# abstract-liu/LORB_SLAM

Hardware: AMD Instinct MI355X
Metric: ORB matches/sec + local-BA iterations/sec (50 KF, 10k pts) at 1/2/4/8 MI355X (higher is better)
Workload: dtype f64+u8; 1 GPU; c4_local_mapping_step_chained; windows_per_gpu=1, kf=50, fixed_kf=5, points=10679, observations=75130, new_kf_keypoints=2000, match=2000x~10679 bf crossCheck, parallelism=independent windows x1

## Files before the change

### lorb_slam_amd/csrc/lorb_ba.hip

```cpp
#ifndef LORB_NO_CONTRACT
#pragma clang fp contract(fast)
#endif
#include "lorb_ba_math.h"
#include "lorb_internal.h"
#include "lorb_ba_dev.h"
#include "lorb_ba_plan.h"

#include <algorithm>
#include <cmath>
#include <type_traits>

namespace {

using namespace lorb::ba;
using lorb::residual;
using lorb::residual_jac;
using lorb::residual_jac_s;
using lorb::residual_s;

__device__ __forceinline__ void init_run(const BaDev& d, int W, int ctot, int n_pt, int nf, const LMOpt& o, const int i,
                                         const int stride) {
  if (i < W) {
    WinState s;
    s.radius = o.init_radius; s.decrease_factor = 2.0; s.cost = 0.0; s.x_norm = 0.0; s.gmax = 0.0;
// ... 1453 lines not shown
    const int n = std::max(std::max(std::max(P->W, P->Ctot), P->NF), std::min(3 * P->pt_launch, 256 * 1024));
    hipLaunchKernelGGL(k_ba_init, dim3(lorb::ceil_div(std::max(n, 1), 256)), dim3(256), 0, ctx->stream, P->dev, P->W,
                       P->Ctot, P->pt_launch, P->NF, o);
  }
  LORB_CHECK_LAUNCH(ctx);
  if (o.max_iter <= 0) return enqueue_linearize(P, o);
  for (int it = 0; it < o.max_iter; ++it) LORB_TRY(enqueue_iteration(P, o, it == 0, it + 1 == o.max_iter));
  return LORB_OK;
}

int plan_solve(lorb_ba_plan* P, const lorb_lm_options* opt) {
  lorb_ctx* ctx = P->ctx;
  LMOpt o = to_dev_opt(opt);
  P->fold = fold_of(P);
  const bool timing = ctx->ktime || no_graph() || (P->comm && !P->comm->rccl);
  if (timing) return enqueue_solve(P, o);
  const lorb_ba_plan::GraphKey key = graph_key(P);
  const bool same = key == P->gkey && same_opt(P->graph_opt, o);
  return P->cache.replay_or_capture(ctx, same, [&] { return enqueue_solve(P, o); },
                                    [&] { P->gkey = key; P->graph_opt = o; });
}

int plan_read(lorb_ba_plan* P, double* const* pose_out, double* const* point_out,
              lorb_ba_summary* sums) {
  lorb_ctx* ctx = P->ctx;
  std::vector<WinState> st(P->W);
  std::vector<std::vector<double>> hp(P->W);
  LORB_HIP(ctx, hipMemcpyAsync(st.data(), P->d_state, sizeof(WinState) * P->W, hipMemcpyDeviceToHost, ctx->stream));
  LORB_HIP(ctx, hipStreamSynchronize(ctx->stream));
  for (int w = 0; w < P->W; ++w) {
    const BaWin& bw = P->hwin[w];
    const int cur = st[w].cur;
// ... 10 lines not shown
      if (bw.n_obs_all == 0) { s.iterations = 0; s.termination = LORB_TERM_FUNCTION_TOL; }
      sums[w] = s;
    }
  }
  LORB_HIP(ctx, hipStreamSynchronize(ctx->stream));
  for (int w = 0; w < P->W; ++w) {
    if (hp[w].empty()) continue;
    const std::vector<int>& map = P->cam_map[w];
    for (int c = 0; c < P->hwin[w].n_poses; ++c)
      for (int q = 0; q < 6; ++q)
        pose_out[w][6 * (size_t)c + q] = hp[w][6 * (size_t)(map.empty() ? c : map[c]) + q];
  }
  return LORB_OK;
}

}

struct lorb_ba_group {
  lorb_ctx* ctx = nullptr;
  std::vector<lorb_ba_plan*> plans;
  GraphCache cache{"group graph"};
  LMOpt graph_opt{};
  std::vector<unsigned> gens;
  std::vector<lorb_ba_plan::GraphKey> keys;
  int n_fused = 0;
};

namespace {

bool group_fused(const lorb_ba_group* G) {
// ... 343 lines not shown
```

### lorb_slam_amd/csrc/lorb_ba_build.hip

```cpp
#ifndef LORB_NO_CONTRACT
#pragma clang fp contract(fast)
#endif
#include "lorb_ba_math.h"
#include "lorb_internal.h"
#include "lorb_ba_dev.h"
#include "lorb_ba_plan.h"

#include <algorithm>
#include <chrono>
#include <cmath>
#include <map>

struct lorb_ba_devbuild {
  int K_cap = 0, P_cap = 0, C = 0, F = 0, Wd = 0;
  int* key_out = nullptr; int* val_out = nullptr;
  int* scr = nullptr; size_t scr_bytes = 0;
  int* pt_cnt = nullptr;
  int* hdr = nullptr;
  int* cov = nullptr;
  int* cam_cnt = nullptr;
  unsigned long long* bits = nullptr;
  int* perm = nullptr;
  int pblk_cap = 0, part_cap = 0, gspan_cap = 0, sgrp_cap = 0;
  size_t gpart_cap = 0;
  int* pinned = nullptr; size_t pinned_n = 0;
  bool dirty = true;
  bool sorted_hint = false;
  std::vector<double> h_red;
  unsigned char* up_dev = nullptr; unsigned char* up_host = nullptr; int up_bp_cap = 0;
  const unsigned char* up_host_dev = nullptr;
  size_t off_live = 0, off_perm = 0, off_gcam = 0, off_bp = 0, up_bytes = 0;
  std::vector<char> last_adj;
  std::vector<int> h_copy;
  std::vector<int> last_map;
  hipEvent_t rb_ev = nullptr;
  bool rb_pending = false, rb_sorted = false, rb_fuse = false;
  ~lorb_ba_devbuild() {
    if (rb_ev) (void)hipEventDestroy(rb_ev);
    if (pinned) (void)hipHostFree(pinned);
    if (up_host) (void)hipHostFree(up_host);
  }
};

namespace {

using namespace lorb::ba;

void print_diagnostics(const lorb_ba_plan& p) {
  if (p.hp_n)
// ... 715 lines not shown
    const unsigned long long bal = __ballot(pr);
    const unsigned msk = half ? (unsigned)(bal >> 32) : (unsigned)bal;
    if (n > 0) {
      if (msk) {
        const int f = __builtin_ctz(msk);
        hi = lo + (int)(((long long)n * (f + 1)) / 33);
        if (f > 0) lo = lo + (int)(((long long)n * f) / 33) + 1;
      } else {
        lo = lo + (int)(((long long)n * 32) / 33) + 1;
      }
    }
  }
  s0 = __shfl(lo, 0, 64);
  s1 = __shfl(lo, 32, 64);
}
__global__ __launch_bounds__(256) void k_db_gather(lorb_ba_window_dev w, BaDev d, int K, const int* __restrict__ key,
                                                   const int* __restrict__ val, DbFused f, DbCams cams) {
  const int gt = blockIdx.x * 256 + threadIdx.x, gs = gridDim.x * 256;
  for (int i = gt; i < f.up_words; i += gs) f.up_dst[i] = f.up_src[i];
  const int* __restrict__ perm = cams.perm;
  const int* __restrict__ gcam = cams.gcam;
  {
    const int m = max(max(6 * f.C, 6 * f.F), 3 * f.P);
    for (int i = gt; i < m; i += gs) {
      if (i < 6 * f.C) {
        const int c = i / 6, q = i - 6 * c;
        d.x_init_pose[6 * perm[c] + q] = (double)w.d_pose_init[i];
        if (q == 0) const_cast<int*>(d.cam_active)[perm[c]] = gcam[c] > 0;
      }
      if (i < 6 * f.F) const_cast<double*>(d.fixed_pose)[i] = (double)w.d_fixed_pose[i];
      if (i < 3 * f.P) d.x_init_pt[i] = (double)w.d_point_init[i];
    }
  }
  for (int g = gt >> 6; g < f.G; g += gs >> 6) {
    int s0, s1;
    group_bounds(d.pt_obs_off, f.P, (long long)g * f.S, (long long)(g + 1) * f.S, threadIdx.x & 63, s0, s1);
    if ((threadIdx.x & 63) == 0) {
      PBlk b;
      b.win = 0; b.p0 = s0; b.cnt = s1 - s0; b.o0 = d.pt_obs_off[s0]; b.no = d.pt_obs_off[s1] - d.pt_obs_off[s0];
      const_cast<PBlk*>(d.pblk)[g] = b;
    }
  }
  for (int i = gt; i < f.nsg; i += gs) f.sgrp[i] = make_int4(0, i * f.sgf, min(f.sgf, f.G - i * f.sgf), 0);
// ... 101 lines not shown
  P->hwin.assign(1, BaWin{});
  P->pt_launch = b.P_cap;
  return LORB_OK;
}

int up_alloc(lorb_ba_plan* P, int bp_need) {
  lorb_ba_devbuild& b = *P->devb;
  if (b.up_dev && b.up_bp_cap >= bp_need) return LORB_OK;
  lorb_ctx* ctx = P->ctx;
  const int cap = std::max(bp_need + bp_need / 4, 16);
  auto al = [](size_t x) { return (x + 255) & ~(size_t)255; };
  const size_t C = (size_t)std::max(b.C, 1);
  b.off_live = al(sizeof(BaWin));
  b.off_perm = b.off_live + 256;
  b.off_gcam = b.off_perm + al(4 * C);
  b.off_bp = b.off_gcam + al(4 * C);
  b.up_bytes = b.off_bp + sizeof(BlockPair) * (size_t)cap;
  if (b.up_dev) {
    LORB_TRY(dfree(P, b.up_dev));
    (void)hipHostFree(b.up_host);
    b.up_host = nullptr;
  }
  LORB_TRY(dalloc(P, b.up_bytes, &b.up_dev));
  LORB_HIP(ctx, hipHostMalloc(reinterpret_cast<void**>(&b.up_host), b.up_bytes));
  LORB_HIP(ctx, hipHostGetDevicePointer((void**)&b.up_host_dev, b.up_host, 0));
  b.up_bp_cap = cap;
  BaDev& d = P->dev;
  d.win = reinterpret_cast<const BaWin*>(b.up_dev);
  d.live = reinterpret_cast<const int*>(b.up_dev + b.off_live);
  b.perm = reinterpret_cast<int*>(b.up_dev + b.off_perm);
  d.bp = reinterpret_cast<const BlockPair*>(b.up_dev + b.off_bp);
  P->grid_bp = cap;
// ... 140 lines not shown
                           shape_ok ? "another rank" : "this rank", w->n_poses, b.C, w->n_fixed, b.F);
  if (gerr & 64)
    return phase_rc != LORB_OK ? phase_rc
                               : lorb::set_error(ctx, LORB_E_DEVICE, "device plan build failed on another rank");
  if (gerr & 8) return lorb::set_error(ctx, LORB_E_INVALID, "live point / observation count outside [0, capacity] (%d / %d)",
                                       b.P_cap, b.K_cap);
  if (gerr & 1) return lorb::set_error(ctx, LORB_E_INVALID, "observation with a point index outside [0, n_points)");
  if (gerr & 2) return lorb::set_error(ctx, LORB_E_INVALID, "observation with a frame index >= n_poses");
  if (gerr & 4) return lorb::set_error(ctx, LORB_E_INVALID, "a point observed twice by one camera");
  if ((gerr & 16) || Pn < 0 || Pn > b.P_cap) return lorb::set_error(ctx, LORB_E_INVALID, "n_points %d outside [0, %d]", Pn, b.P_cap);
  if (kGB - gmaxk < 1)
    return lorb::set_error(ctx, LORB_E_UNSUPPORTED, "a point with %d observations (device plans hold <= %d)", gmaxk, kGB - 1);
  return LORB_OK;
}

void db_camera_order(lorb_ba_devbuild& b, const DbBuild& r) {
  const int C = b.C;
  bool same_adj = b.last_adj.size() == (size_t)C * C;
  for (int i = 0; i < C && same_adj; ++i) {
    const int* row = r.gcov + (size_t)i * C;
    const char* last = b.last_adj.data() + (size_t)i * C;
    for (int j = 0; j < C; ++j)
      if (last[j] != (char)((i == j && r.gcam[i] > 0) || row[j] > 0)) { same_adj = false; break; }
  }
  if (!same_adj) {
    std::vector<char> adj((size_t)C * C, 0);
    for (int i = 0; i < C; ++i)
      for (int j = 0; j < C; ++j) adj[(size_t)i * C + j] = (i == j && r.gcam[i] > 0) || r.gcov[(size_t)i * C + j] > 0;
    b.last_map = camera_order(C, adj);
    b.last_adj.swap(adj);
  }
}

void db_blocks(const lorb_ba_devbuild& b, DbBuild& r) {
  const int C = b.C;
  std::vector<int> inv(C), fc(C);
  for (int c = 0; c < C; ++c) inv[b.last_map[c]] = c;
  for (int ch = 0; ch < C; ++ch) {
    fc[ch] = ch;
    for (int cl = 0; cl <= ch; ++cl) {
      const int cnt = ch == cl ? r.cam_cnt[inv[ch]] : r.cov[(size_t)inv[ch] * C + inv[cl]];
      if (ch != cl && r.gcov[(size_t)inv[ch] * C + inv[cl]] > 0) fc[ch] = std::min(fc[ch], cl);
      if (ch != cl && cnt == 0) continue;
      r.bps.push_back(BlockPair{0, ch, cl, r.n_pairs, cnt});
      r.n_pairs += cnt;
    }
// ... 41 lines not shown
  P->grid_sg = b.pblk_cap;
  return up_alloc(P, (int)r.bps.size());
}

void db_stage_and_gather(lorb_ctx* ctx, const lorb_ba_window_dev* w, lorb_ba_plan* P, const DbBuild& r, HostPhase& hp) {
  lorb_ba_devbuild& b = *P->devb;
  const std::vector<int>& map = b.last_map;
  const std::vector<BlockPair>& bps = r.bps;
  const int C = b.C;
  unsigned char* h = b.up_host;
  memcpy(h, &P->hwin[0], sizeof(BaWin));
  const int live[3] = {r.G, (int)bps.size(), r.NSG};
  memcpy(h + b.off_live, live, sizeof(live));
  memcpy(h + b.off_perm, map.data(), sizeof(int) * C);
  memcpy(h + b.off_gcam, r.gcam, sizeof(int) * C);
  if (!bps.empty()) memcpy(h + b.off_bp, bps.data(), sizeof(BlockPair) * bps.size());
  const int up_words = (int)((b.off_bp + sizeof(BlockPair) * bps.size() + 3) / 4);
  hp.mark(4);
  DbFused f{C, b.F, r.Pn, r.G, r.S, P->env_total, C * b.Wd, b.rb_sorted ? 1 : 0, b.bits, b.hdr, b.cov, C * C + C,
            reinterpret_cast<const int*>(b.up_host_dev), reinterpret_cast<int*>(b.up_dev), up_words};
  f.sgf = r.SF; f.nsg = r.NSG; f.sgrp = const_cast<int4*>(P->dev.sgrp);
  DbCams cams;
  for (int c = 0; c < C; ++c) { cams.perm[c] = map[c]; cams.gcam[c] = r.gcam[c]; }
  const int NB = lorb::ceil_div(r.K, 256);
  hipLaunchKernelGGL(k_db_gather, dim3(std::max(NB, 1)), dim3(256), 0, ctx->stream, *w, P->dev, r.K, b.key_out, b.val_out,
                     f, cams);
  b.dirty = false;
  hp.mark(5);
}

int dev_build_finish(lorb_ctx* ctx, const lorb_ba_window_dev* w, lorb_ba_plan* P, int lerr) {
  lorb_ba_devbuild& b = *P->devb;
  const int phase_rc = (lerr || !b.rb_pending) ? LORB_OK : db_phase1_wait(ctx, w, P);
  static const bool hp_log = env_flag("LORB_HOST_PHASE");
  HostPhase hp{P, hp_log};
  DbBuild r;
  LORB_TRY(db_land(ctx, w, P, lerr, phase_rc, r));
  hp.mark(0);
  db_camera_order(b, r);
  hp.mark(1);
  P->cam_map.assign(1, b.last_map);
  db_blocks(b, r);
  LORB_TRY(db_layout(ctx, w, P, r));
  hp.mark(2);
  LORB_TRY(db_buffers(P, r));
  hp.mark(3);
  db_stage_and_gather(ctx, w, P, r, hp);
  LORB_CHECK_LAUNCH(ctx);
  return LORB_OK;
}

int dev_build(lorb_ctx* ctx, const lorb_ba_window_dev* w, lorb_ba_plan* P) {
  int lerr = 0;
  LORB_TRY(dev_build_issue(ctx, w, P, &lerr));
  return dev_build_finish(ctx, w, P, lerr);
}

int create_host_plan(lorb_ctx* ctx, lorb_comm* comm, int32_t n_windows, const lorb_ba_window* windows, lorb_ba_plan** out) {
  if (!ctx || !out || n_windows < 0 || (n_windows > 0 && !windows)) return LORB_E_INVALID;
  if (comm && comm->ctx != ctx) return lorb::set_error(ctx, LORB_E_INVALID, "communicator belongs to another context");
  *out = nullptr;
  lorb_ba_plan* P = new (std::nothrow) lorb_ba_plan();
  if (!P) return LORB_E_NOMEM;
// ... 33 lines not shown
  print_diagnostics(*this);
  delete devb;
  for (void* p : allocs) (void)hipFree(p);
}

namespace lorb {
int ba_plan_update_dev_issue(lorb_ba_plan* P, const lorb_ba_window_dev* w) {
  if (!P || !w || !P->devb || P->comm) return LORB_E_INVALID;
  int lerr = 0;
  return dev_build_issue(P->ctx, w, P, &lerr);
}
int ba_plan_update_dev_finish(lorb_ba_plan* P, const lorb_ba_window_dev* w) {
  if (!P || !w || !P->devb || P->comm) return LORB_E_INVALID;
  return dev_build_finish(P->ctx, w, P, 0);
}
void ba_plan_sorted_hint(lorb_ba_plan* P, bool sorted) {
  if (P && P->devb) P->devb->sorted_hint = sorted;
}
const int* ba_plan_point_offsets(const lorb_ba_plan* P) { return P && P->devb ? P->dev.pt_obs_off : nullptr; }
void ba_plan_window_counts(const lorb_ba_plan* P, int* n_points, int* n_obs) {
  *n_points = P->Ptot;
  *n_obs = P->K;
}

static dim3 result_grid(const lorb_ba_plan* P) {
  return dim3(lorb::ceil_div(std::max(std::max(6 * P->Ctot, 1), std::min(3 * P->Ptot, 256 * 1024)), 256));
}
int ba_plan_result_ring_dev(lorb_ba_plan* P, float* ring, int R, int t0, float* d_point_out) {
  if (!P || !P->devb || !ring || R < 1) return LORB_E_INVALID;
  hipLaunchKernelGGL(k_db_result, result_grid(P), dim3(256), 0, P->ctx->stream, P->dev, P->Ctot, P->Ptot,
// ... 64 lines not shown
```

### lorb_slam_amd/csrc/lorb_ba_plan.h

```cpp
#pragma once
#include "lorb_ba_dev.h"

#include <algorithm>
#include <cstring>
#include <vector>

namespace lorb::ba {

inline bool env_flag(const char* name) { const char* e = getenv(name); return e && e[0] == '1'; }

inline size_t dbg_words(size_t windows, size_t stamp_slots) {
#ifdef LORB_CHOL_TRACE
  return windows * 512;
#elif defined(LORB_LS_STAMPS)
  return stamp_slots * 8;
#else
  return windows * 8;
#endif
}

struct GraphCache {
  const char* what;
  hipGraph_t graph = nullptr;
  hipGraphExec_t exec = nullptr;
// ... 57 lines not shown
  double hp_us = 0.0, hp_sec[6] = {};
  int hp_n = 0;
  std::vector<lorb::ba::BaWin> hwin;
  std::vector<void*> allocs;
  lorb::ba::BaDev dev{};
  lorb::ba::WinState* d_state = nullptr;
  lorb::ba::GraphCache cache{"graph"};
  lorb::ba::LMOpt graph_opt{};
  unsigned gen = 0;
  struct GraphKey {
    int kind = -1, lds = 0, memset_env = 0, env_total = 0, grid_pblk = 0, grid_bp = 0, pt_launch = 0, x2_n = 0;
    int red_wide = 0, sup = 0, grid_sg = 0;
    int fold = 0;
    bool operator==(const GraphKey& o) const { return memcmp(this, &o, sizeof(GraphKey)) == 0; }
  } gkey;
  int grid_pblk = 0, grid_bp = 0;
  int grid_sg = 0;
  bool has_super = false;
  bool fold = false;
  int pt_launch = 0;
  int* live = nullptr;
  lorb_comm* comm = nullptr;
  double *x2_send = nullptr, *x2_recv = nullptr;
  size_t fx_n = 0;
  size_t x2_off = 0;
  std::vector<std::vector<int>> cam_map;
  int chol_kind = -1;
  lorb_ba_devbuild* devb = nullptr;
  ~lorb_ba_plan();
};
// ... 1 lines not shown
```

### lorb_slam_amd/csrc/lorb_internal.h

```cpp
#pragma once

#include <hip/hip_runtime.h>

#include <cstdarg>
#include <cstdint>
#include <cstdio>
#include <cstring>
#include <new>
#include <string>
#include <vector>

#include "../../include/lorb_c.h"

struct lorb_ctx {
  int device = 0;
  hipStream_t stream = nullptr;
  std::string err;
  hipEvent_t ev[64] = {};
  static constexpr int kScratch = 128;
  void* scratch[kScratch] = {};
  size_t scratch_sz[kScratch] = {};
  std::vector<unsigned char> up_mirror[kScratch];
  bool ktime = false;
  std::vector<hipEvent_t> kev_pool;
// ... 58 lines not shown
  } while (0)

#define LORB_CHECK_LAUNCH(ctx) LORB_HIP(ctx, hipGetLastError())

#define LORB_TRY(expr)          \
  do {                          \
    int rc_ = (expr);           \
    if (rc_ != LORB_OK) return rc_; \
  } while (0)

int ba_plan_result64_dev(lorb_ba_plan* P, double* d_out);
int ba_plan_result_ring_dev(lorb_ba_plan* P, float* ring, int R, int t0, float* d_point_out);
void ba_plan_sorted_hint(lorb_ba_plan* P, bool sorted);
int ba_plan_update_dev_issue(lorb_ba_plan* P, const lorb_ba_window_dev* w);
int ba_plan_update_dev_finish(lorb_ba_plan* P, const lorb_ba_window_dev* w);
void ba_plan_window_counts(const lorb_ba_plan* P, int* n_points, int* n_obs);
const int* ba_plan_point_offsets(const lorb_ba_plan* P);

int match1_keys_dev(lorb_ctx* ctx, const uint8_t* d_q, int nq, const uint8_t* d_t, int nt,
                    unsigned long long** qkey_out, hipStream_t stream = nullptr);
int match1_keys_into(lorb_ctx* ctx, const uint8_t* d_q, int nq, const uint8_t* d_t, int nt,
                     unsigned long long* qkey, uint32_t* tkey, hipStream_t st);

int scratch(lorb_ctx* ctx, int slot, size_t bytes, void** out);
template <typename T>
int scratch_t(lorb_ctx* ctx, int slot, size_t count, T** out) {
  void* p = nullptr;
  int rc = scratch(ctx, slot, count * sizeof(T) + 16, &p);
  *out = static_cast<T*>(p);
  return rc;
// ... 567 lines not shown
```

### lorb_slam_amd/csrc/lorb_map.hip

```cpp
#include <algorithm>
#include <chrono>
#include <cstdlib>

#include "lorb_internal.h"

namespace {

struct MapDev {
  float* pos; uint8_t* desc; int* obs_pt; int* obs_kf; float* obs_uv;
  float* pos2; uint8_t* desc2; int* obs_pt2; int* obs_kf2; float* obs_uv2;
  int* obs_frame;
  int* cnt;
  int* flag_pt; int* newid; int* flag_obs; int* newpos;
  int* flag_new; int* newnew;
  int* tile_tot;
  float* ring;
  float* pose_init; float* fixed;
  int P_cap, K_cap, W, F, R;
};

struct Pose6 { float v[6]; };

__device__ __forceinline__ int ring_slot(int kf, int R) { const int r = kf % R; return r < 0 ? r + R : r; }

// ... 239 lines not shown
  double prof_ms[8] = {};
  int prof_n = 0;
  std::chrono::steady_clock::time_point prof_clk{};
  int* mt = nullptr;
  unsigned long long* qkey = nullptr;
  uint32_t* tkey = nullptr;
  int* pinned = nullptr;
  lorb_ba_plan* plan = nullptr;
  bool plan_ok = false;
  bool broken = false;
  bool overlap = false;
  hipStream_t side = nullptr;
  hipEvent_t ev_built = nullptr, ev_app = nullptr;
  bool built = false;
  int n_overlapped = 0;
  std::vector<void*> allocs;
  ~lorb_map() {
    if (prof && prof_n)
      fprintf(stderr, "lorb_map profile over %d steps (ms/step): match %.3f unproject %.3f append %.3f slide %.3f "
              "plan %.3f solve %.3f writeback %.3f\n", prof_n, prof_ms[0] / prof_n, prof_ms[1] / prof_n,
              prof_ms[2] / prof_n, prof_ms[3] / prof_n, prof_ms[4] / prof_n, prof_ms[5] / prof_n, prof_ms[6] / prof_n);
    if (side) (void)hipStreamSynchronize(side);
    if (plan) (void)lorb_ba_plan_destroy(plan);
    if (pinned) (void)hipHostFree(pinned);
    if (ev_built) (void)hipEventDestroy(ev_built);
    if (ev_app) (void)hipEventDestroy(ev_app);
    if (side) (void)hipStreamDestroy(side);
    for (void* p : allocs) (void)hipFree(p);
  }
};
// ... 160 lines not shown
  return LORB_OK;
}

int map_build_fail(lorb_map* M, int rc) {
  M->built = false;
  hipStream_t s = M->ctx->stream;
  if (hipMemcpyAsync(M->pinned, M->m.cnt, sizeof(int) * 8, hipMemcpyDeviceToHost, s) == hipSuccess &&
      hipStreamSynchronize(s) == hipSuccess) {
    M->h_P = M->pinned[0]; M->h_K = M->pinned[1];
  } else {
    M->broken = true;
  }
  return rc;
}

int map_build_done(lorb_map* M) {
  lorb_ctx* ctx = M->ctx;
  M->plan_ok = true;
  if (!M->ev_built) LORB_HIP(ctx, hipEventCreateWithFlags(&M->ev_built, hipEventDisableTiming));
  LORB_HIP(ctx, hipEventRecord(M->ev_built, ctx->stream));
  M->built = true;
  LORB_TRY(map_mark(M, 4));
  lorb::ba_plan_window_counts(M->plan, &M->h_P, &M->h_K);
  return LORB_OK;
}

int map_prepare(lorb_map* M, const lorb_frame_params* frame, const float pose[6], const float Tcw[16], int32_t n,
                const uint8_t* d_desc, const float* d_x, const float* d_y, const float* d_depth, bool split = false) {
  if (!M || !frame || !pose || !Tcw || n < 0) return LORB_E_INVALID;
  lorb_ctx* ctx = M->ctx;
  if (n > M->n_cap) return lorb::set_error(ctx, LORB_E_INVALID, "%d keypoints > the map's max_keypoints %d", n, M->n_cap);
  if (n > 0 && (!d_desc || !d_x || !d_y || !d_depth)) return LORB_E_INVALID;
  if (M->broken) return lorb::set_error(ctx, LORB_E_DEVICE, "the map is unusable after an earlier failed step");
  hipStream_t s = ctx->stream;
  MapDev& m = M->m;
  const int kf = M->t0 + m.W;
  M->prof_clk = std::chrono::steady_clock::now();
  auto mark = [&](int i) { return map_mark(M, i); };
  LORB_TRY(mark(7));
  const bool ovl = M->overlap && M->built && !M->prof && !ctx->ktime;
  if (ovl && !M->side) {
    LORB_HIP(ctx, hipStreamCreateWithFlags(&M->side, hipStreamNonBlocking));
    LORB_HIP(ctx, hipEventCreateWithFlags(&M->ev_app, hipEventDisableTiming));
// ... 39 lines not shown
    LORB_HIP(ctx, hipStreamSynchronize(s));
    if (M->pinned[2] & 1)
      return lorb::set_error(ctx, LORB_E_NOMEM, "map capacity exceeded (points %d + %d new / %d, observations %d + %d new / %d)",
                             M->h_P, n, m.P_cap, M->h_K, n, m.K_cap);
  }
  LORB_TRY(mark(2));
  LORB_TRY(map_slide(M, M->t0 + 1, std::min(M->h_P + n, m.P_cap), std::min(M->h_K + n, m.K_cap), M->h_K, M->h_P,
                      M->plan_ok ? lorb::ba_plan_point_offsets(M->plan) : nullptr));
  LORB_TRY(mark(3));
  const lorb_ba_window_dev w = window_of(M);
  M->plan_ok = false;
  if (split) {
    if (const int rc = lorb::ba_plan_update_dev_issue(M->plan, &w); rc != LORB_OK) return map_build_fail(M, rc);
    return LORB_OK;
  }
  if (const int rc = lorb_ba_plan_update_dev(M->plan, &w); rc != LORB_OK) return map_build_fail(M, rc);
  return map_build_done(M);
}

int map_build_finish(lorb_map* M) {
  const lorb_ba_window_dev w = window_of(M);
  if (const int rc = lorb::ba_plan_update_dev_finish(M->plan, &w); rc != LORB_OK) return map_build_fail(M, rc);
  return map_build_done(M);
}

int map_finish(lorb_map* M) {
  LORB_TRY(lorb::ba_plan_result_ring_dev(M->plan, M->m.ring, M->m.R, M->t0, M->m.pos));
  LORB_TRY(map_mark(M, 6));
  if (M->prof) M->prof_n++;
  return LORB_OK;
}

// ... 3 lines not shown
struct lorb_map_group {
  std::vector<lorb_map*> maps;
  std::vector<lorb_ba_group*> bag;
  int n_steps_fused = 0;
  ~lorb_map_group() {
    for (lorb_ba_group* g : bag) (void)lorb_ba_group_destroy(g);
  }
};

extern "C" {

int lorb_map_step_dev(lorb_map* M, const lorb_frame_params* frame, const float pose[6], const float Tcw[16], int32_t n,
                      const uint8_t* d_desc, const float* d_x, const float* d_y, const float* d_depth,
                      const lorb_lm_options* opt) {
  if (!M || !opt) return LORB_E_INVALID;
  LORB_TRY(map_prepare(M, frame, pose, Tcw, n, d_desc, d_x, d_y, d_depth));
  LORB_TRY(lorb_ba_plan_solve(M->plan, opt));
  LORB_TRY(map_mark(M, 5));
  return map_finish(M);
}

int lorb_map_set_overlap(lorb_map* M, int32_t enable) {
  if (!M || (enable != 0 && enable != 1)) return LORB_E_INVALID;
  M->overlap = enable == 1;
  if (!M->overlap && M->side) {
    LORB_HIP(M->ctx, hipStreamSynchronize(M->side));
  }
  return LORB_OK;
}

int lorb_map_counts(lorb_map* M, int32_t* out, int32_t n) {
  if (!M || !out || n < 0) return LORB_E_INVALID;
  lorb_ctx* ctx = M->ctx;
  LORB_HIP(ctx, hipMemcpyAsync(M->pinned, M->m.cnt, sizeof(int) * 8, hipMemcpyDeviceToHost, ctx->stream));
  LORB_HIP(ctx, hipStreamSynchronize(ctx->stream));
  const int32_t v[9] = {M->pinned[0], M->pinned[1], M->t0, M->last_n, M->pinned[3], M->pinned[4], M->pinned[5], M->m.W,
                        M->n_overlapped};
  for (int i = 0; i < n && i < 9; ++i) out[i] = v[i];
  return LORB_OK;
}

int lorb_map_read(lorb_map* M, const lorb_map_state* st) {
  if (!M || !st) return LORB_E_INVALID;
  lorb_ctx* ctx = M->ctx;
  hipStream_t s = ctx->stream;
  const MapDev& m = M->m;
  int32_t c[8];
  LORB_TRY(lorb_map_counts(M, c, 8));
  const size_t P = (size_t)c[0], K = (size_t)c[1];
  auto down = [&](void* h, const void* d, size_t bytes) -> int {
    if (h && bytes) LORB_HIP(ctx, hipMemcpyAsync(h, d, bytes, hipMemcpyDeviceToHost, s));
    return LORB_OK;
  };
// ... 120 lines not shown
```

### lorb_slam_amd/runtime.py

```python
import ctypes as C
import os

import numpy as np

from . import _abi as A

_HERE = os.path.dirname(os.path.abspath(__file__))
LIB_PATH = os.environ.get("LORB_LIB_PATH") or os.path.join(_HERE, "liblorb.so")
_lib = None


class LorbError(RuntimeError):
    pass


def lib():
    global _lib
    if _lib is None:
        if not os.path.exists(LIB_PATH):
            raise LorbError(f"{LIB_PATH} not built: run `make -C lorb_slam_amd/csrc` (hipcc, gfx950)")
        L = C.CDLL(LIB_PATH)
        L.lorb_last_error.restype = C.c_char_p
        L.lorb_last_error.argtypes = [C.c_void_p]
        for name in ("lorb_create", "lorb_destroy", "lorb_sync", "lorb_malloc", "lorb_free",
# ... 402 lines not shown
        pp = (A.f64p * 1)(A.ptr(poses, C.c_double))
        qp = (A.f64p * 1)(A.ptr(pts, C.c_double))
        summ = (A.BASummary * 1)()
        self.ctx.check(lib().lorb_ba_plan_read(self._p, pp, qp, summ), "lorb_ba_plan_read")
        return [poses], [pts[:info["points"]]], [summ[0].as_dict()]

    def result_dev(self, d_pose, d_points):
        self.ctx.check(lib().lorb_ba_plan_result_dev(self._p, d_pose.ptr if d_pose is not None else None,
                                                     d_points.ptr if d_points is not None else None),
                       "lorb_ba_plan_result_dev")


class LocalMap:

    COUNT_KEYS = ("points", "observations", "t0", "keypoints", "new_points", "new_observations", "matches", "window",
                  "overlapped_steps")

    def __init__(self, ctx, init, max_points=None, max_obs=None, max_keypoints=4096):
        self.ctx, self._keep = ctx, A.KeepAlive()
        k = self._keep.keep
        s = A.MapInit()
        s.n_window, s.n_fixed = len(init["pose_init"]), len(init["fixed_pose"])
        s.n_points, s.n_obs = len(init["point_init"]), len(init["obs_point"])
        s.max_points = int(max_points or 2 * s.n_points + 8 * max_keypoints)
        s.max_obs = int(max_obs or 2 * s.n_obs + 8 * max_keypoints)
        s.max_keypoints = int(max_keypoints)
        s.fx, s.fy, s.cx, s.cy = (float(v) for v in init["intr"])
        s.pose = A.ptr(k(A.f32(init["pose_init"])), C.c_float)
        s.fixed_pose = A.ptr(k(A.f32(init["fixed_pose"]).reshape(-1, 6)), C.c_float)
        s.point = A.ptr(k(A.f32(init["point_init"])), C.c_float)
        s.point_desc = A.ptr(k(A.u8(init["point_desc"])), C.c_uint8)
# ... 15 lines not shown
                                               C.c_int32(n), d_desc.ptr, d_x.ptr, d_y.ptr, d_depth.ptr, C.byref(opt)),
                       "lorb_map_step_dev")

    def step(self, fp, kf, opt=None):
        fps = A.make_frame_params(fp) if isinstance(fp, dict) else fp
        arrs = [self.ctx.to_device(A.u8(kf["desc"])), self.ctx.to_device(A.f32(kf["x"])),
                self.ctx.to_device(A.f32(kf["y"])), self.ctx.to_device(A.f32(kf["depth"]))]
        try:
            self.step_dev(fps, kf["pose"], kf["Tcw"], len(kf["x"]), *arrs, opt=opt)
            self.ctx.sync()
        finally:
            for a in arrs:
                a.free()

    def counts(self):
        v = (C.c_int32 * 9)()
        self.ctx.check(lib().lorb_map_counts(self._p, v, C.c_int32(9)), "lorb_map_counts")
        return dict(zip(self.COUNT_KEYS, [int(x) for x in v]))

    def read(self):
        c = self.counts()
        P, K = c["points"], c["observations"]
        out = dict(point=np.zeros((max(P, 1), 3), np.float32), point_desc=np.zeros((max(P, 1), 32), np.uint8),
                   obs_point=np.zeros(max(K, 1), np.int32), obs_kf=np.zeros(max(K, 1), np.int32),
                   obs_uv=np.zeros((max(K, 1), 2), np.float32), obs_frame=np.zeros(max(K, 1), np.int32),
                   pose=np.zeros((self.W, 6), np.float32), fixed_pose=np.zeros((max(self.F, 1), 6), np.float32),
                   match_train=np.zeros(max(c["keypoints"], 1), np.int32))
        summ = A.BASummary()
        st = A.MapState()
        st.point = A.ptr(out["point"], C.c_float); st.point_desc = A.ptr(out["point_desc"], C.c_uint8)
        st.obs_point = A.ptr(out["obs_point"], C.c_int32); st.obs_kf = A.ptr(out["obs_kf"], C.c_int32)
        st.obs_uv = A.ptr(out["obs_uv"], C.c_float); st.obs_frame = A.ptr(out["obs_frame"], C.c_int32)
# ... 111 lines not shown
```

Baseline: 11580 BA iterations/s.

## Speculatively reuse previous BA block structure to overlap device build with solve

In the chained map step, the BA plan build no longer waits on the host readback. It speculatively assumes the camera adjacency and block-pair structure match the previous step. A single-block device kernel checks adjacency and capacity on the GPU and recomputes block-pair offsets, then the gather and the solve are enqueued right away. The host verifies the speculation after the solve is enqueued and falls back to a full rebuild and re-solve on a miss, which adds extra work and complexity whenever the structure changes.

```diff
diff --git a/lorb_slam_amd/csrc/lorb_ba.hip b/lorb_slam_amd/csrc/lorb_ba.hip
--- a/lorb_slam_amd/csrc/lorb_ba.hip
+++ b/lorb_slam_amd/csrc/lorb_ba.hip
@@ -1491,8 +1491,9 @@
   LMOpt o = to_dev_opt(opt);
   P->fold = fold_of(P);
   const bool timing = ctx->ktime || no_graph() || (P->comm && !P->comm->rccl);
+  const lorb_ba_plan::GraphKey key = graph_key(P);
+  P->skey = key;
   if (timing) return enqueue_solve(P, o);
-  const lorb_ba_plan::GraphKey key = graph_key(P);
   const bool same = key == P->gkey && same_opt(P->graph_opt, o);
   return P->cache.replay_or_capture(ctx, same, [&] { return enqueue_solve(P, o); },
                                     [&] { P->gkey = key; P->graph_opt = o; });
@@ -1533,6 +1534,16 @@
   return LORB_OK;
 }
 
+}
+
+namespace lorb {
+bool ba_plan_solve_key_same(lorb_ba_plan* P) {
+  const bool fold_was = P->fold;
+  P->fold = fold_of(P);
+  const bool same = graph_key(P) == P->skey;
+  P->fold = fold_was;
+  return same;
+}
 }
 
 struct lorb_ba_group {
diff --git a/lorb_slam_amd/csrc/lorb_ba_build.hip b/lorb_slam_amd/csrc/lorb_ba_build.hip
--- a/lorb_slam_amd/csrc/lorb_ba_build.hip
+++ b/lorb_slam_amd/csrc/lorb_ba_build.hip
@@ -29,10 +29,14 @@
   std::vector<double> h_red;
   unsigned char* up_dev = nullptr; unsigned char* up_host = nullptr; int up_bp_cap = 0;
   const unsigned char* up_host_dev = nullptr;
-  size_t off_live = 0, off_perm = 0, off_gcam = 0, off_bp = 0, up_bytes = 0;
+  size_t off_live = 0, off_perm = 0, off_gcam = 0, off_adj = 0, off_bp = 0, up_bytes = 0;
+  bool spec_ok = false, spec_pending = false;
+  int spec_sf = 1;
+  int* spec_out = nullptr;
   std::vector<char> last_adj;
   std::vector<int> h_copy;
   std::vector<int> last_map;
+  std::vector<lorb::ba::BlockPair> last_bps;
   hipEvent_t rb_ev = nullptr;
   bool rb_pending = false, rb_sorted = false, rb_fuse = false;
   ~lorb_ba_devbuild() {
@@ -778,9 +782,78 @@
   s0 = __shfl(lo, 0, 64);
   s1 = __shfl(lo, 32, 64);
 }
+struct DbSpec {
+  int C, P_cap, K_cap, pblk_cap, nbp, sf, sg_force, part_stride;
+  long long gpart_cap;
+  const int* hdr; const int* cov; const int* cam_cnt;
+  const unsigned char* adj;
+  BaWin* win; int* live; BlockPair* bp; int* cam_active;
+  int* out;
+};
+__global__ __launch_bounds__(1024) void k_db_spec(DbSpec s, DbCams cams) {
+  __shared__ int s_inv[kPmSpan];
+  __shared__ int s_sum[1024];
+  __shared__ int s_bad;
+  const int t = threadIdx.x, C = s.C;
+  if (t == 0) s_bad = 0;
+  if (t < C) s_inv[cams.perm[t]] = t;
+  __syncthreads();
+  int K = s.hdr[0], Pn = s.hdr[3];
+  const int maxk = s.hdr[1], err = s.hdr[2];
+  bool ok = err == 0 && K >= 0 && K <= s.K_cap && Pn >= 0 && Pn <= s.P_cap && maxk >= 0 && maxk <= kGB - 1;
+  int S = 1, G = 0, NSG = 0;
+  if (ok) {
+    S = kGB - maxk;
+    G = Pn > 0 ? (int)(((long long)K + Pn - 1) / S) + 1 : 0;
+    const int SF = s.sg_force ? (G > 1 ? s.sg_force : 1) : (G > 512 ? (G + 479) / 480 : 1);
+    NSG = G > 0 ? (G + SF - 1) / SF : 0;
+    ok = G <= s.pblk_cap && SF == s.sf && (long long)NSG * s.part_stride <= s.gpart_cap;
+  }
+  bool bad = false;
+  for (int k = t; k < C * C; k += 1024) {
+    const int i = k / C, j = k - i * C;
+    if (j <= i) bad |= ((i == j ? s.cam_cnt[i] : s.cov[k]) > 0) != (s.adj[k] != 0);
+  }
+  if (bad) s_bad = 1;
+  __syncthreads();
+  ok = ok && !s_bad;
+  if (!ok) { K = 0; Pn = 0; G = 0; NSG = 0; S = 1; }
+  if (t == 0) {
+    s.out[0] = ok; s.out[1] = K; s.out[2] = Pn; s.out[3] = G; s.out[4] = S; s.out[5] = NSG;
+    s.win->n_points = Pn; s.win->n_obs = K; s.win->n_obs_all = K; s.win->n_pblk = G; s.win->n_sg = NSG;
+    s.live[0] = G; s.live[1] = ok ? s.nbp : 0; s.live[2] = NSG;
+  }
+  if (!ok) return;
+  if (t < C) s.cam_active[cams.perm[t]] = s.cam_cnt[t] > 0;
+  const int per = (s.nbp + 1023) / 1024, b0 = min(t * per, s.nbp), b1 = min(b0 + per, s.nbp);
+  int sum = 0;
+  for (int k = b0; k < b1; ++k) {
+    const int a = s_inv[s.bp[k].ch], b = s_inv[s.bp[k].cl];
+    sum += a == b ? s.cam_cnt[a] : s.cov[max(a, b) * C + min(a, b)];
+  }
+  s_sum[t] = sum;
+  __syncthreads();
+  for (int o = 1; o < 1024; o <<= 1) {
+    const int v = t >= o ? s_sum[t - o] : 0;
+    __syncthreads();
+    s_sum[t] += v;
+    __syncthreads();
+  }
+  int off = s_sum[t] - sum;
+  for (int k = b0; k < b1; ++k) {
+    const int a = s_inv[s.bp[k].ch], b = s_inv[s.bp[k].cl];
+    const int cnt = a == b ? s.cam_cnt[a] : s.cov[max(a, b) * C + min(a, b)];
+    s.bp[k].off = off; s.bp[k].cnt = cnt;
+    off += cnt;
+  }
+}
+
+template <bool SPEC>
 __global__ __launch_bounds__(256) void k_db_gather(lorb_ba_window_dev w, BaDev d, int K, const int* __restrict__ key,
-                                                   const int* __restrict__ val, DbFused f, DbCams cams) {
+                                                   const int* __restrict__ val, DbFused f, DbCams cams,
+                                                   const int* __restrict__ spec) {
   const int gt = blockIdx.x * 256 + threadIdx.x, gs = gridDim.x * 256;
+  if (SPEC) { K = spec[1]; f.P = spec[2]; f.G = spec[3]; f.S = spec[4]; f.nsg = spec[5]; }
   for (int i = gt; i < f.up_words; i += gs) f.up_dst[i] = f.up_src[i];
   const int* __restrict__ perm = cams.perm;
   const int* __restrict__ gcam = cams.gcam;
@@ -790,7 +863,7 @@
       if (i < 6 * f.C) {
         const int c = i / 6, q = i - 6 * c;
         d.x_init_pose[6 * perm[c] + q] = (double)w.d_pose_init[i];
-        if (q == 0) const_cast<int*>(d.cam_active)[perm[c]] = gcam[c] > 0;
+        if (!SPEC && q == 0) const_cast<int*>(d.cam_active)[perm[c]] = gcam[c] > 0;
       }
       if (i < 6 * f.F) const_cast<double*>(d.fixed_pose)[i] = (double)w.d_fixed_pose[i];
       if (i < 3 * f.P) d.x_init_pt[i] = (double)w.d_point_init[i];
@@ -922,8 +995,11 @@
   b.off_live = al(sizeof(BaWin));
   b.off_perm = b.off_live + 256;
   b.off_gcam = b.off_perm + al(4 * C);
-  b.off_bp = b.off_gcam + al(4 * C);
+  b.off_adj = b.off_gcam + al(4 * C);
+  b.off_bp = b.off_adj + al(C * C);
   b.up_bytes = b.off_bp + sizeof(BlockPair) * (size_t)cap;
+  b.spec_ok = false;
+  if (!b.spec_out) LORB_TRY(dalloc(P, (size_t)8, &b.spec_out));
   if (b.up_dev) {
     LORB_TRY(dfree(P, b.up_dev));
     (void)hipHostFree(b.up_host);
@@ -1094,7 +1170,7 @@
   return LORB_OK;
 }
 
-void db_camera_order(lorb_ba_devbuild& b, const DbBuild& r) {
+bool db_camera_order(lorb_ba_devbuild& b, const DbBuild& r) {
   const int C = b.C;
   bool same_adj = b.last_adj.size() == (size_t)C * C;
   for (int i = 0; i < C && same_adj; ++i) {
@@ -1110,6 +1186,7 @@
     b.last_map = camera_order(C, adj);
     b.last_adj.swap(adj);
   }
+  return same_adj;
 }
 
 void db_blocks(const lorb_ba_devbuild& b, DbBuild& r) {
@@ -1181,6 +1258,7 @@
   memcpy(h + b.off_live, live, sizeof(live));
   memcpy(h + b.off_perm, map.data(), sizeof(int) * C);
   memcpy(h + b.off_gcam, r.gcam, sizeof(int) * C);
+  if (!b.last_adj.empty()) memcpy(h + b.off_adj, b.last_adj.data(), b.last_adj.size());
   if (!bps.empty()) memcpy(h + b.off_bp, bps.data(), sizeof(BlockPair) * bps.size());
   const int up_words = (int)((b.off_bp + sizeof(BlockPair) * bps.size() + 3) / 4);
   hp.mark(4);
@@ -1190,14 +1268,73 @@
   DbCams cams;
   for (int c = 0; c < C; ++c) { cams.perm[c] = map[c]; cams.gcam[c] = r.gcam[c]; }
   const int NB = lorb::ceil_div(r.K, 256);
-  hipLaunchKernelGGL(k_db_gather, dim3(std::max(NB, 1)), dim3(256), 0, ctx->stream, *w, P->dev, r.K, b.key_out, b.val_out,
-                     f, cams);
+  hipLaunchKernelGGL(k_db_gather<false>, dim3(std::max(NB, 1)), dim3(256), 0, ctx->stream, *w, P->dev, r.K, b.key_out,
+                     b.val_out, f, cams, (const int*)nullptr);
   b.dirty = false;
   hp.mark(5);
 }
 
+void spec_spoil(lorb_ba_devbuild& b) {
+  if (env_flag("LORB_SPEC_SPOIL") && b.last_adj.size() > 1) b.last_adj[1] ^= 1;
+}
+
+bool spec_allowed(const lorb_ctx* ctx, const lorb_ba_plan* P) {
+  const lorb_ba_devbuild& b = *P->devb;
+  return !P->comm && b.spec_ok && b.sorted_hint && b.C > 0 && !ctx->ktime && !env_flag("LORB_NO_SPEC");
+}
+
+int dev_spec_issue(lorb_ctx* ctx, const lorb_ba_window_dev* w, lorb_ba_plan* P, int obs_hint) {
+  lorb_ba_devbuild& b = *P->devb;
+  const int C = b.C;
+  DbCams cams;
+  for (int c = 0; c < C; ++c) { cams.perm[c] = b.last_map[c]; cams.gcam[c] = 0; }
+  const char* e = getenv("LORB_SG_F");
+  const BaWin& hw = P->hwin[0];
+  DbSpec s{C, w->max_points, w->max_obs, b.pblk_cap, (int)b.last_bps.size(), b.spec_sf, e && atoi(e) >= 1 ? atoi(e) : 0,
+           hw.part_stride, (long long)b.gpart_cap, b.hdr, b.cov, b.cam_cnt, b.up_dev + b.off_adj,
+           reinterpret_cast<BaWin*>(b.up_dev), reinterpret_cast<int*>(b.up_dev + b.off_live),
+           reinterpret_cast<BlockPair*>(b.up_dev + b.off_bp), const_cast<int*>(P->dev.cam_active), b.spec_out};
+  hipLaunchKernelGGL(k_db_spec, dim3(1), dim3(1024), 0, ctx->stream, s, cams);
+  DbFused f{C, b.F, 0, 0, 1, P->env_total, C * b.Wd, 1, b.bits, b.hdr, b.cov, C * C + C, nullptr, nullptr, 0};
+  f.sgf = b.spec_sf; f.nsg = 0; f.sgrp = const_cast<int4*>(P->dev.sgrp);
+  const int NB = lorb::ceil_div(std::min(std::max(obs_hint, 1), std::max(w->max_obs, 1)), 256);
+  hipLaunchKernelGGL(k_db_gather<true>, dim3(NB), dim3(256), 0, ctx->stream, *w, P->dev, 0, b.key_out, b.val_out, f, cams,
+                     (const int*)b.spec_out);
+  LORB_CHECK_LAUNCH(ctx);
+  b.spec_pending = true;
+  return LORB_OK;
+}
+
+int dev_spec_verify(lorb_ctx* ctx, const lorb_ba_window_dev* w, lorb_ba_plan* P, bool* hit) {
+  lorb_ba_devbuild& b = *P->devb;
+  *hit = false;
+  b.spec_pending = false;
+  b.spec_ok = false;
+  b.rb_pending = false;
+  LORB_HIP(ctx, lorb::spin_wait(b.rb_ev));
+  if (b.pinned[2] & 16) return LORB_OK;
+  const int bw_was = P->hwin[0].bw;
+  DbBuild r;
+  LORB_TRY(db_land(ctx, w, P, 0, LORB_OK, r));
+  if (!db_camera_order(b, r)) return LORB_OK;
+  db_blocks(b, r);
+  bool same = r.bw == bw_was && r.bps.size() == b.last_bps.size();
+  for (size_t i = 0; same && i < r.bps.size(); ++i) same = r.bps[i].ch == b.last_bps[i].ch && r.bps[i].cl == b.last_bps[i].cl;
+  if (!same) return LORB_OK;
+  LORB_TRY(db_layout(ctx, w, P, r));
+  if (r.SF != b.spec_sf || r.G > b.pblk_cap || (size_t)std::max(r.part_total, 1ll) > b.gpart_cap ||
+      (int)r.bps.size() > b.up_bp_cap || !lorb::ba_plan_solve_key_same(P))
+    return LORB_OK;
+  b.last_bps.swap(r.bps);
+  b.dirty = false;
+  b.spec_ok = true;
+  *hit = true;
+  return LORB_OK;
+}
+
 int dev_build_finish(lorb_ctx* ctx, const lorb_ba_window_dev* w, lorb_ba_plan* P, int lerr) {
   lorb_ba_devbuild& b = *P->devb;
+  b.spec_ok = b.spec_pending = false;
   const int phase_rc = (lerr || !b.rb_pending) ? LORB_OK : db_phase1_wait(ctx, w, P);
   static const bool hp_log = env_flag("LORB_HOST_PHASE");
   HostPhase hp{P, hp_log};
@@ -1214,6 +1351,9 @@
   hp.mark(3);
   db_stage_and_gather(ctx, w, P, r, hp);
   LORB_CHECK_LAUNCH(ctx);
+  b.last_bps.swap(r.bps);
+  b.spec_sf = r.SF;
+  b.spec_ok = !P->comm;
   return LORB_OK;
 }
 
@@ -1277,6 +1417,24 @@
   if (!P || !w || !P->devb || P->comm) return LORB_E_INVALID;
   return dev_build_finish(P->ctx, w, P, 0);
 }
+int ba_plan_update_dev_spec(lorb_ba_plan* P, const lorb_ba_window_dev* w, int obs_hint, bool* speculated) {
+  if (!P || !w || !P->devb || !speculated) return LORB_E_INVALID;
+  *speculated = false;
+  lorb_ctx* ctx = P->ctx;
+  lorb_ba_devbuild& b = *P->devb;
+  if (!spec_allowed(ctx, P)) return dev_build(ctx, w, P);
+  spec_spoil(b);
+  int lerr = 0;
+  LORB_TRY(dev_build_issue(ctx, w, P, &lerr));
+  if (!(b.rb_sorted && b.rb_fuse)) return dev_build_finish(ctx, w, P, lerr);
+  LORB_TRY(dev_spec_issue(ctx, w, P, obs_hint));
+  *speculated = true;
+  return LORB_OK;
+}
+int ba_plan_update_dev_verify(lorb_ba_plan* P, const lorb_ba_window_dev* w, bool* hit) {
+  if (!P || !w || !P->devb || !hit || !P->devb->spec_pending) return LORB_E_INVALID;
+  return dev_spec_verify(P->ctx, w, P, hit);
+}
 void ba_plan_sorted_hint(lorb_ba_plan* P, bool sorted) {
   if (P && P->devb) P->devb->sorted_hint = sorted;
 }
diff --git a/lorb_slam_amd/csrc/lorb_ba_plan.h b/lorb_slam_amd/csrc/lorb_ba_plan.h
--- a/lorb_slam_amd/csrc/lorb_ba_plan.h
+++ b/lorb_slam_amd/csrc/lorb_ba_plan.h
@@ -95,6 +95,7 @@
     int fold = 0;
     bool operator==(const GraphKey& o) const { return memcmp(this, &o, sizeof(GraphKey)) == 0; }
   } gkey;
+  GraphKey skey;
   int grid_pblk = 0, grid_bp = 0;
   int grid_sg = 0;
   bool has_super = false;
diff --git a/lorb_slam_amd/csrc/lorb_internal.h b/lorb_slam_amd/csrc/lorb_internal.h
--- a/lorb_slam_amd/csrc/lorb_internal.h
+++ b/lorb_slam_amd/csrc/lorb_internal.h
@@ -96,6 +96,9 @@
 void ba_plan_sorted_hint(lorb_ba_plan* P, bool sorted);
 int ba_plan_update_dev_issue(lorb_ba_plan* P, const lorb_ba_window_dev* w);
 int ba_plan_update_dev_finish(lorb_ba_plan* P, const lorb_ba_window_dev* w);
+int ba_plan_update_dev_spec(lorb_ba_plan* P, const lorb_ba_window_dev* w, int obs_hint, bool* speculated);
+int ba_plan_update_dev_verify(lorb_ba_plan* P, const lorb_ba_window_dev* w, bool* hit);
+bool ba_plan_solve_key_same(lorb_ba_plan* P);
 void ba_plan_window_counts(const lorb_ba_plan* P, int* n_points, int* n_obs);
 const int* ba_plan_point_offsets(const lorb_ba_plan* P);
 
diff --git a/lorb_slam_amd/csrc/lorb_map.hip b/lorb_slam_amd/csrc/lorb_map.hip
--- a/lorb_slam_amd/csrc/lorb_map.hip
+++ b/lorb_slam_amd/csrc/lorb_map.hip
@@ -277,6 +277,8 @@
   hipEvent_t ev_built = nullptr, ev_app = nullptr;
   bool built = false;
   int n_overlapped = 0;
+  bool spec = false;
+  int n_spec = 0, n_fallback = 0;
   std::vector<void*> allocs;
   ~lorb_map() {
     if (prof && prof_n)
@@ -467,19 +469,25 @@
   return rc;
 }
 
-int map_build_done(lorb_map* M) {
+int map_built_event(lorb_map* M) {
   lorb_ctx* ctx = M->ctx;
-  M->plan_ok = true;
   if (!M->ev_built) LORB_HIP(ctx, hipEventCreateWithFlags(&M->ev_built, hipEventDisableTiming));
   LORB_HIP(ctx, hipEventRecord(M->ev_built, ctx->stream));
   M->built = true;
+  return LORB_OK;
+}
+
+int map_build_done(lorb_map* M) {
+  M->plan_ok = true;
+  LORB_TRY(map_built_event(M));
   LORB_TRY(map_mark(M, 4));
   lorb::ba_plan_window_counts(M->plan, &M->h_P, &M->h_K);
   return LORB_OK;
 }
 
 int map_prepare(lorb_map* M, const lorb_frame_params* frame, const float pose[6], const float Tcw[16], int32_t n,
-                const uint8_t* d_desc, const float* d_x, const float* d_y, const float* d_depth, bool split = false) {
+                const uint8_t* d_desc, const float* d_x, const float* d_y, const float* d_depth, bool split = false,
+                bool may_spec = false) {
   if (!M || !frame || !pose || !Tcw || n < 0) return LORB_E_INVALID;
   lorb_ctx* ctx = M->ctx;
   if (n > M->n_cap) return lorb::set_error(ctx, LORB_E_INVALID, "%d keypoints > the map's max_keypoints %d", n, M->n_cap);
@@ -549,8 +557,38 @@
     if (const int rc = lorb::ba_plan_update_dev_issue(M->plan, &w); rc != LORB_OK) return map_build_fail(M, rc);
     return LORB_OK;
   }
+  if (may_spec && M->built && !M->prof) {
+    const int obs_hint = std::min(M->h_K + n, m.K_cap);
+    if (const int rc = lorb::ba_plan_update_dev_spec(M->plan, &w, obs_hint, &M->spec); rc != LORB_OK) {
+      M->spec = false;
+      return map_build_fail(M, rc);
+    }
+    if (M->spec) {
+      M->n_spec++;
+      return map_built_event(M);
+    }
+    return map_build_done(M);
+  }
   if (const int rc = lorb_ba_plan_update_dev(M->plan, &w); rc != LORB_OK) return map_build_fail(M, rc);
   return map_build_done(M);
+}
+
+int map_spec_verify(lorb_map* M, const lorb_lm_options* opt) {
+  M->spec = false;
+  const lorb_ba_window_dev w = window_of(M);
+  bool hit = false;
+  if (const int rc = lorb::ba_plan_update_dev_verify(M->plan, &w, &hit); rc != LORB_OK) return map_build_fail(M, rc);
+  if (!hit) {
+    M->n_fallback++;
+    if (const int rc = lorb_ba_plan_update_dev(M->plan, &w); rc != LORB_OK) return map_build_fail(M, rc);
+  }
+  M->plan_ok = true;
+  lorb::ba_plan_window_counts(M->plan, &M->h_P, &M->h_K);
+  if (!hit) {
+    LORB_TRY(map_built_event(M));
+    LORB_TRY(lorb_ba_plan_solve(M->plan, opt));
+  }
+  return LORB_OK;
 }
 
 int map_build_finish(lorb_map* M) {
@@ -584,8 +622,13 @@
                       const uint8_t* d_desc, const float* d_x, const float* d_y, const float* d_depth,
                       const lorb_lm_options* opt) {
   if (!M || !opt) return LORB_E_INVALID;
-  LORB_TRY(map_prepare(M, frame, pose, Tcw, n, d_desc, d_x, d_y, d_depth));
-  LORB_TRY(lorb_ba_plan_solve(M->plan, opt));
+  LORB_TRY(map_prepare(M, frame, pose, Tcw, n, d_desc, d_x, d_y, d_depth, false, true));
+  if (const int rc = lorb_ba_plan_solve(M->plan, opt); rc != LORB_OK) {
+    if (!M->spec) return rc;
+    M->spec = false;
+    return map_build_fail(M, rc);
+  }
+  if (M->spec) LORB_TRY(map_spec_verify(M, opt));
   LORB_TRY(map_mark(M, 5));
   return map_finish(M);
 }
@@ -604,9 +647,9 @@
   lorb_ctx* ctx = M->ctx;
   LORB_HIP(ctx, hipMemcpyAsync(M->pinned, M->m.cnt, sizeof(int) * 8, hipMemcpyDeviceToHost, ctx->stream));
   LORB_HIP(ctx, hipStreamSynchronize(ctx->stream));
-  const int32_t v[9] = {M->pinned[0], M->pinned[1], M->t0, M->last_n, M->pinned[3], M->pinned[4], M->pinned[5], M->m.W,
-                        M->n_overlapped};
-  for (int i = 0; i < n && i < 9; ++i) out[i] = v[i];
+  const int32_t v[11] = {M->pinned[0], M->pinned[1], M->t0, M->last_n, M->pinned[3], M->pinned[4], M->pinned[5], M->m.W,
+                         M->n_overlapped, M->n_spec, M->n_fallback};
+  for (int i = 0; i < n && i < 11; ++i) out[i] = v[i];
   return LORB_OK;
 }
 
diff --git a/lorb_slam_amd/runtime.py b/lorb_slam_amd/runtime.py
--- a/lorb_slam_amd/runtime.py
+++ b/lorb_slam_amd/runtime.py
@@ -440,7 +440,7 @@
 class LocalMap:
 
     COUNT_KEYS = ("points", "observations", "t0", "keypoints", "new_points", "new_observations", "matches", "window",
-                  "overlapped_steps")
+                  "overlapped_steps", "speculated_builds", "spec_fallbacks")
 
     def __init__(self, ctx, init, max_points=None, max_obs=None, max_keypoints=4096):
         self.ctx, self._keep = ctx, A.KeepAlive()
@@ -486,8 +486,8 @@
                 a.free()
 
     def counts(self):
-        v = (C.c_int32 * 9)()
-        self.ctx.check(lib().lorb_map_counts(self._p, v, C.c_int32(9)), "lorb_map_counts")
+        v = (C.c_int32 * len(self.COUNT_KEYS))()
+        self.ctx.check(lib().lorb_map_counts(self._p, v, C.c_int32(len(v))), "lorb_map_counts")
         return dict(zip(self.COUNT_KEYS, [int(x) for x in v]))
 
     def read(self):
```

Result: faster. 11720 BA iterations/s (median of 6 runs) (+1.2%).
